# rpl-cmu/bevrender

Measured on AMD Instinct MI355X. Metric: samples/sec fwd+bwd, 6-cam 256x704 BEV-lift+corr, higher is better.
Workload: dtype bf16; 1 GPU; cfg3: 6-cam 256x704 features (64x64x176), 200x200 BEV, C=64 h=2 D=5, L=2 encoder layers (TSA+SCA), T=2 (1 no-grad history frame(s) + 1 fwd+bwd), correlation head with contrastive + lifted-structure losses, AdamW; batch 8 per GPU; backbone/render CNN excluded; global_batch=8, per_gpu_batch=8, parallelism=dp1

## Files before the change

bevrender_amd/csrc/attn_gather_fwd.hip:

```cpp
#include "attn_tap.h"
#include "attn_host.h"

#ifndef BEVR_GATHER_ROWS
#define BEVR_GATHER_ROWS 0
#endif
#ifndef BEVR_GATHER_X3
#define BEVR_GATHER_X3 0
#endif

#include "bevr_prof.h"

BEVR_PROF_DEFINE(gather, 32)

namespace {

constexpr int GT = 32;
constexpr int NT = GT / 32;
constexpr int ROWS = 256;
constexpr int PITCH = 272;
constexpr int WIN_COLS = 28;
constexpr int STRIP_KEYS = WIN_COLS / 2;
template <int NP> struct LdsGn {
  static constexpr int K_IMG = GT * 64, V_IMG = GT * 32, W_IMG = (GT / 16) * 2 * 64 * 16;
  static constexpr int OFF_K = 0;
  static constexpr int OFF_VLO = NP * K_IMG;
  static constexpr int OFF_VHI = OFF_VLO + NP * V_IMG;
  static constexpr int OFF_W = OFF_VHI + NP * V_IMG;
  static constexpr int W_BYTES = NP * W_IMG;
  static constexpr int OFF_OFF = OFF_W + W_BYTES;
  static constexpr int OFF_CT = OFF_OFF + GT * 4;
  static constexpr int OFF_FD = OFF_CT + 16;
  static constexpr int BUF = OFF_FD + WIN_COLS * 8;
  static constexpr int WIN_PLANE = WIN_COLS * PITCH * 4;
  static constexpr int WIN = NP * WIN_PLANE;
  static constexpr int OFF_WIN = 2 * BUF;
  static constexpr int TOTAL = OFF_WIN + 2 * WIN;
};
typedef LdsGn<BEVR_GATHER_X3 ? 2 : 1> LdsG;
static_assert(LdsG::BUF % 16 == 0 && LdsG::WIN % 16 == 0, "16-byte aligned LDS blocks");
static_assert((BEVR_GATHER_X3 ? 1 : 2) * LdsG::TOTAL <= 160 * 1024, "workgroups per CU");
static_assert(LdsG::WIN_PLANE + 2 * QB * 4 < 65536, "the lo plane of a tap is an immediate offset of its hi plane's read");
__device__ __forceinline__ int w_image_pos(int n) {
  const int m = n >> 3, half = (n >> 2) & 1, dd = n & 3;
  return (m * 64 + n + 32 * half) * 16 + dd * 4;
}
__device__ __forceinline__ void barrier_lds() { asm volatile("s_waitcnt lgkmcnt(0)\n\ts_barrier" ::: "memory"); }
__device__ __forceinline__ void wait_vm0() { asm volatile("s_waitcnt vmcnt(0)" ::: "memory"); }
constexpr float RAISE = 40.0f;
constexpr float F16_RAISE = 15.0f;
constexpr float F16_LIFT = 8.0f;
constexpr float F16_PMAX_PER_KEY = 6.103515625e-05f;

template <int V> struct IntC { static constexpr int value = V; };
typedef const char __attribute__((address_space(1)))* gptr_t;
typedef char __attribute__((address_space(3)))* lptr_t;
__device__ __forceinline__ void glds16(const char* src, char* lds_base) {
  __builtin_amdgcn_global_load_lds((gptr_t)src, (lptr_t)lds_base, 16, 0, 0);
}

#if BEVR_DROP
static_assert(BEVR_GATHER_ROWS && !BEVR_GATHER_X3, "the keep mask: the 16-bit row-range kernels");
#define BEVR_GATHER_KERNEL attn_gather_fwd_drop_kernel
#define BEVR_GATHER_ROW_PARAMS , const int row0, const int n_rows, const unsigned drop_thr, const unsigned drop_seed
#define BEVR_GATHER_WAVES_PER_SIMD 4
#elif BEVR_GATHER_X3
#define BEVR_GATHER_KERNEL attn_gather_fwd_x3_kernel
#define BEVR_GATHER_ROW_PARAMS , const int row0, const int n_rows
#define BEVR_GATHER_WAVES_PER_SIMD 2
#elif BEVR_GATHER_ROWS
#define BEVR_GATHER_KERNEL attn_gather_fwd_rows_kernel
#define BEVR_GATHER_ROW_PARAMS , const int row0, const int n_rows
#define BEVR_GATHER_WAVES_PER_SIMD 4
#else
#define BEVR_GATHER_KERNEL attn_gather_fwd_kernel
#define BEVR_GATHER_ROW_PARAMS
#define BEVR_GATHER_WAVES_PER_SIMD 4
#endif
template <int PREC, int NB, bool EXACT, bool DMA>
__global__ __launch_bounds__(512, BEVR_GATHER_WAVES_PER_SIMD) void BEVR_GATHER_KERNEL(
    bevr_attn_desc d, const char* __restrict__ Q, const char* __restrict__ K, const char* __restrict__ V,
    const char* __restrict__ key_ws, const uint32_t* __restrict__ table_pk, const float* __restrict__ mref,
    float* __restrict__ O, float* __restrict__ LSE, int* __restrict__ flags BEVR_GATHER_ROW_PARAMS) {
  constexpr bool BAND = BEVR_GATHER_ROWS != 0;
  constexpr bool X3 = tap_split(PREC);
  static_assert(X3 == (BEVR_GATHER_X3 != 0), "the split mode lives in its own translation unit");
  static_assert(!X3 || BAND, "the split mode takes a row range");
  constexpr int NP = tap_np<PREC>;
  constexpr int ROWB = X3 ? 128 : 64;
  typedef TapHalf<PREC> H16;
#if !BEVR_GATHER_ROWS
  constexpr int row0 = 0, n_rows = 0;
#endif
  typedef LdsG L;
  extern __shared__ __attribute__((aligned(16))) char smem[];

  const int n_ph = d.n_prob * d.heads;
  const int xcd = blockIdx.x & 7, slot = blockIdx.x >> 3;
  const int ph = (slot / d.S) * 8 + xcd;
  if (ph >= n_ph) return;
  const int j = slot % d.S;
  if constexpr (EXACT) {
    if (flags[ph * d.S + j] == 0) return;
  }
  const int prob = ph / d.heads, hd = ph % d.heads;
  const int tid = threadIdx.x, n_wave = blockDim.x >> 6;
  const int wave = __builtin_amdgcn_readfirstlane(tid >> 6), lane = tid & 63;
  const int li = lane & 15, kg = lane >> 4;
  const int Mp = d.S * d.Sp;
  const int nblk = ((BAND ? n_rows : d.S) + QB - 1) / QB;
  const int rows_q = nblk * QB;
  const int row_end = BAND ? row0 + n_rows : d.S;
  const bool to_end = !BAND || row_end == d.S;
  const float rx = (float)(d.Wt - 1) / (2.0f * (float)(d.S - 1));
  const float jrx = (float)j * rx;
  const unsigned smem_base = (unsigned)(size_t)(lptr_t)smem;

  const char* tbl = reinterpret_cast<const char*>(table_pk + (size_t)hd * d.Wp * d.Hp);
  const unsigned lane16 = (unsigned)lane * 16u;
  const size_t tbl_plane = (size_t)d.heads * d.Wp * d.Hp * 4;
  auto fill_one = [&](char* win, int c, int xc, int r0) {
    static_assert(ROWS == 256, "one 16-byte load per lane and column");
    BEVR_ASSERT(c >= 0 && c < WIN_COLS && xc >= 0 && xc < d.Wp && r0 >= 0 && (DMA ? r0 + ROWS <= d.Hp : r0 < d.Hp));
    if constexpr (DMA) {
      const char* sbase = tbl + ((size_t)__builtin_amdgcn_readfirstlane(xc) * d.Hp + __builtin_amdgcn_readfirstlane(r0)) * 4;
      glds16(sbase + lane16, win + (c * PITCH) * 4);
      if constexpr (X3) glds16(sbase + tbl_plane + lane16, win + L::WIN_PLANE + (c * PITCH) * 4);
    } else {
      const int rr = r0 + 4 * lane;
#pragma unroll
      for (int pl = 0; pl < NP; ++pl) {
        const char* src = tbl + pl * tbl_plane + ((size_t)xc * d.Hp + rr) * 4;
        u32x4 v = {0u, 0u, 0u, 0u};
#pragma unroll
        for (int k = 0; k < 4; ++k)
          if (rr + k < d.Hp) v[k] = *reinterpret_cast<const uint32_t*>(src + 4 * k);
        *reinterpret_cast<u32x4*>(win + pl * L::WIN_PLANE + (c * PITCH) * 4 + lane * 16) = v;
      }
    }
  };
  auto fill_share = [&](const int* fd, char* win, int nfill) {
    for (int c = wave; c < nfill; c += n_wave) fill_one(win, c, fd[2 * c], fd[2 * c + 1]);
  };

  for (int i = tid; i < 2 * L::W_BYTES / 16; i += (int)blockDim.x)
    *reinterpret_cast<u32x4*>(smem + (i / (L::W_BYTES / 16)) * L::BUF + L::OFF_W + (i % (L::W_BYTES / 16)) * 16) =
        u32x4{0u, 0u, 0u, 0u};
  if (wave == n_wave - 1) {
    __builtin_amdgcn_s_setprio(3);
    const int pg = prob * d.groups + hd / (d.heads / d.groups);
    const KeyW* kws = reinterpret_cast<const KeyW*>(key_ws) + (size_t)pg * d.Np;
    const StepBox* box = reinterpret_cast<const StepBox*>(key_ws + key_ws_box_offset(d)) + (size_t)pg * (d.Np / 32);
    const char* Kp = K + (size_t)ph * d.Np * ROWB;
    const char* Vp = V + (size_t)ph * d.Np * ROWB;
    const int n_steps = d.Np / GT;

    struct Em {
      unsigned long long sel;
      int step, nfill, fd_xc, fd_r0, koff;
      u32x2 w[NP];
    };
    int step = -1;
    unsigned long long rem = 0ull;
    const int kl = lane & (GT - 1);
    const bool klane = lane < GT;
    KeyW kw_n = kws[kl];
    StepBox sb0_n = box[0], sb1_n = box[NT - 1];
    int ar = 0, xc = 0, x0 = 0, a0w = 0, cols = 0;
    bool fits = false;
    u32x2 w_t[NP];
#pragma unroll
    for (int pl = 0; pl < NP; ++pl) w_t[pl] = u32x2{0u, 0u};
    auto advance = [&](Em& em) -> bool {
      while (rem == 0ull) {
        if (++step >= n_steps) return false;
        const KeyW kw = kw_n;
        const StepBox sb = box_union(sb0_n, sb1_n);
        if (step + 1 < n_steps) {
          kw_n = kws[(size_t)(step + 1) * GT + kl];
          sb0_n = box[NT * (step + 1)];
          sb1_n = box[NT * (step + 1) + NT - 1];
        }
        if (sb.amax < sb.amin) continue;
        const bool live = klane && step * GT + kl < d.N;
        ar = (kw.aoff >> 3) - d.x_off * d.Hp;
        if constexpr (BAND) ar += row0;
        const float tx = jrx + kw.b;
        const float xf = floorf(tx);
        xc = (int)xf + d.x_off;
        const float fx = tx - xf, fy = kw.fy;
        if constexpr (X3) {
          TAP_SPLIT2((1.0f - fx) * (1.0f - fy), (1.0f - fx) * fy, w_t[0][0], w_t[NP - 1][0]);
          TAP_SPLIT2(fx * (1.0f - fy), fx * fy, w_t[0][1], w_t[NP - 1][1]);
        } else {
          w_t[0][0] = H16::pack2((1.0f - fx) * (1.0f - fy), (1.0f - fx) * fy);
          w_t[0][1] = H16::pack2(fx * (1.0f - fy), fx * fy);
        }
        x0 = (int)floorf(jrx + sb.bmin) + d.x_off;
        const int x1 = (int)floorf(jrx + sb.bmax) + 1 + d.x_off;
        cols = x1 - x0 + 1;
        fits = cols <= WIN_COLS && sb.amax - sb.amin + rows_q + 1 <= ROWS;
        a0w = max(0, min(sb.amin + d.y_off + (BAND ? row0 : 0), d.Hp - ROWS));
        rem = __ballot(live);
      }
      em.w[0] = w_t[0];
      if constexpr (X3) em.w[NP - 1] = w_t[NP - 1];
      em.step = step;
      if (fits) {
        em.sel = rem;
        em.koff = ((xc - x0) * PITCH + (ar - a0w)) * 4;
        em.nfill = cols;
        em.fd_xc = x0 + lane;
        em.fd_r0 = a0w;
      } else {
        const int rank = __builtin_popcountll(rem & ((1ull << kl) - 1ull));
        const bool mine = klane && (rem >> kl & 1ull) && rank < STRIP_KEYS;
        em.sel = __ballot(mine);
        const int akw = max(0, min(ar, d.Hp - ROWS));
        em.koff = (2 * rank * PITCH + (ar - akw)) * 4;
        em.nfill = 2 * __builtin_popcountll(em.sel);
        int src = 0;
        {
          unsigned long long t = em.sel;
          for (int k = 0; k < (lane >> 1) && t; ++k) t &= t - 1;
          src = t ? __builtin_ctzll(t) : 0;
        }
        em.fd_xc = __shfl(xc, src) + (lane & 1);
        em.fd_r0 = __shfl(akw, src);
      }
      rem &= ~em.sel;
      return true;
    };
    auto stage = [&](const Em& em, int e, const Em* nxt) {
      char* bb = smem + (e & 1) * L::BUF;
      const size_t n0 = (size_t)em.step * GT;
#pragma unroll
      for (int i = 0; i < GT / 16; ++i) {
        const int n = 16 * i + (lane >> 2), c = (lane & 3) ^ ((n >> 2) & 3);
        if constexpr (X3) {
          const char* src = Kp + (n0 + n) * ROWB + 64 * (c >> 1) + 16 * (c & 1);
          glds16(src, bb + L::OFF_K + i * 1024);
          glds16(src + 32, bb + L::OFF_K + L::K_IMG + i * 1024);
        } else {
          glds16(Kp + (n0 + n) * 64 + 16 * c, bb + L::OFF_K + i * 1024);
        }
      }
#pragma unroll
      for (int i = 0; i < NT; ++i) {
        const int n = 32 * i + (lane >> 1);
        if constexpr (X3) {
          const char* src = Vp + (n0 + n) * ROWB + 16 * (lane & 1);
          glds16(src, bb + L::OFF_VLO + i * 1024);
          glds16(src + 32, bb + L::OFF_VLO + L::V_IMG + i * 1024);
          glds16(src + 64, bb + L::OFF_VHI + i * 1024);
          glds16(src + 96, bb + L::OFF_VHI + L::V_IMG + i * 1024);
        } else {
          glds16(Vp + (n0 + n) * 64 + 16 * (lane & 1), bb + L::OFF_VLO + i * 1024);
          glds16(Vp + (n0 + n) * 64 + 32 + 16 * (lane & 1), bb + L::OFF_VHI + i * 1024);
        }
      }
      if (klane) {
        char* wk = bb + L::OFF_W + (kl >> 4) * 2048 + w_image_pos(kl & 15);
        *reinterpret_cast<uint32_t*>(wk) = em.w[0][0];
        *reinterpret_cast<uint32_t*>(wk + 256) = em.w[0][1];
        if constexpr (X3) {
          *reinterpret_cast<uint32_t*>(wk + L::W_IMG) = em.w[NP - 1][0];
          *reinterpret_cast<uint32_t*>(wk + L::W_IMG + 256) = em.w[NP - 1][1];
        }
        const bool in = em.sel >> kl & 1ull;
        *reinterpret_cast<unsigned*>(bb + L::OFF_OFF + kl * 4) = smem_base + L::OFF_WIN + (e & 1) * L::WIN + (in ? em.koff : 0);
      }
      if (nxt && lane < nxt->nfill) {
        int* fd = reinterpret_cast<int*>(bb + L::OFF_FD);
        fd[2 * lane] = nxt->fd_xc;
        fd[2 * lane + 1] = nxt->fd_r0;
      }
#if BEVR_DROP
      static_assert(NT == 1, "the third dword (live keys 32..63) carries the emission's first key index");
      if (lane == 0)
        *reinterpret_cast<u32x4*>(bb + L::OFF_CT) =
            u32x4{0u, (unsigned)em.sel, (unsigned)(em.step * GT), nxt ? (unsigned)nxt->nfill : 0u};
#else
      if (lane == 0)
        *reinterpret_cast<u32x4*>(bb + L::OFF_CT) =
            u32x4{0u, (unsigned)em.sel, (unsigned)(em.sel >> 32), nxt ? (unsigned)nxt->nfill : 0u};
#endif
    };

    Em cur, nxt;
    advance(cur);
    bool more = advance(nxt);
    {
      int* fd = reinterpret_cast<int*>(smem + L::BUF + L::OFF_FD);
      if (lane < cur.nfill) {
        fd[2 * lane] = cur.fd_xc;
        fd[2 * lane + 1] = cur.fd_r0;
      }
      if (lane == 0) *reinterpret_cast<u32x4*>(smem + L::BUF + L::OFF_CT) = u32x4{0u, 0u, 0u, (unsigned)cur.nfill};
      barrier_lds();
      fill_share(fd, smem + L::OFF_WIN, cur.nfill);
      stage(cur, 0, more ? &nxt : nullptr);
      wait_vm0();
    }
    PROF_ACC(8);
    for (int e = 0;; ++e) {
      PROF_T_FREE(p0);
      barrier_lds();
      PROF_T_FREE(p1);
      if (!more) {
        if (lane == 0) *reinterpret_cast<u32x4*>(smem + ((e + 1) & 1) * L::BUF + L::OFF_CT) = u32x4{4u, 0u, 0u, 0u};
        barrier_lds();
        break;
      }
      cur = nxt;
      {
        char* wn = smem + L::OFF_WIN + ((e + 1) & 1) * L::WIN;
        for (int c = wave; c < cur.nfill; c += n_wave)
          fill_one(wn, c, __builtin_amdgcn_readlane(cur.fd_xc, c), __builtin_amdgcn_readlane(cur.fd_r0, c));
      }
      PROF_T_FREE(p2);
      more = advance(nxt);
      stage(cur, e + 1, more ? &nxt : nullptr);
      PROF_T_FREE(p3);
      wait_vm0();
      PROF_T_FREE(p4);
      PROF_ADD(4, p1 - p0);
      PROF_ADD(6, p2 - p1);
      PROF_ADD(1, p3 - p2);
      PROF_ADD(3, p4 - p3);
      PROF_ADD(5, 1);
    }
    PROF_FLUSH(gather, 0, lane == 0);
    return;
  }

  const int blk0 = wave * NB;
  const int qb = prob / d.q_div;
  TapOp<NP> qf[NB];
  f32x4 o_lo[NB], o_hi[NB];
  f32x4 negm[NB];
  f32x4 lacc[NB];
  float pmx[NB];
#if BEVR_DROP
  uint32_t hrow[NB];
#endif
  const unsigned qoff0 = (unsigned)(blk0 * QB + li) * 4u + (unsigned)(kg & 1) * (PITCH * 4u);
#pragma unroll
  for (int nb = 0; nb < NB; ++nb) {
    const int row = (BAND ? row0 : 0) + min(blk0 + nb, nblk - 1) * QB + li;
    const size_t mcol = (size_t)j * d.Sp + row;
    if constexpr (X3)
      qf[nb] = tap_ld<NP>(Q + (((size_t)qb * d.heads + hd) * Mp + mcol) * ROWB + 64 * (kg >> 1) + 16 * (kg & 1), 32);
    else
      qf[nb].p[0] = __builtin_bit_cast(
          bf16x8, *reinterpret_cast<const u32x4*>(Q + ((((size_t)qb * d.heads + hd) * Mp + mcol) * 32 + 8 * kg) * 2));
    o_lo[nb] = o_hi[nb] = f32x4{0.f, 0.f, 0.f, 0.f};
    const float mr = EXACT ? 0.f : mref[(size_t)ph * Mp + mcol];
    negm[nb] = f32x4{-mr, -mr, -mr, -mr};
    lacc[nb] = f32x4{0.f, 0.f, 0.f, 0.f};
    pmx[nb] = 0.f;
#if BEVR_DROP
    hrow[nb] = bevr_drop_row(drop_seed, (uint32_t)ph, (uint32_t)mcol);
#endif
  }
  const uint32_t one2 = H16::pack2(1.0f, 1.0f);
  const bf16x8 ones = __builtin_bit_cast(bf16x8, u32x4{one2, one2, one2, one2});
  const int t_off = (4 * kg + (li >> 2)) * 32 + (lane & 3) * 8;
  const int k_off = li * 64 + 16 * (kg ^ (li >> 2));
  typedef const uint32_t __attribute__((address_space(3)))* lds_u32p;
  typedef const volatile uint32_t __attribute__((address_space(3)))* vlds_u32p;

  {
    barrier_lds();
    const int nf0 = __builtin_amdgcn_readfirstlane((int)reinterpret_cast<const u32x4*>(smem + L::BUF + L::OFF_CT)[0][3]);
    fill_share(reinterpret_cast<const int*>(smem + L::BUF + L::OFF_FD), smem + L::OFF_WIN, nf0);
    wait_vm0();
  }
  bool first = true;
  PROF_ACC(8);
  PROF_T_FREE(cprev);
  auto sweep = [&](auto off1_c) {
  constexpr int OFF1 = decltype(off1_c)::value;
  constexpr int NBX = (NB == 2 && OFF1 == 0) ? 1 : NB;
  for (int e = 0;; ++e) {
    PROF_T_FREE(c0);
    barrier_lds();
    PROF_T_FREE(c1);
    PROF_ADD(0, c1 - c0);
    PROF_ADD(4, c0 - cprev);
    PROF_ADD(5, 1);
    PROF_SET(cprev, c1);
    const char* bb = smem + (e & 1) * L::BUF;
    const u32x4 ct = *reinterpret_cast<const u32x4*>(bb + L::OFF_CT);
    if (__builtin_amdgcn_readfirstlane((int)ct[0]) & 4) break;
    fill_share(reinterpret_cast<const int*>(bb + L::OFF_FD), smem + L::OFF_WIN + ((e + 1) & 1) * L::WIN,
               __builtin_amdgcn_readfirstlane((int)ct[3]));
#pragma unroll 1
    for (int t = 0; t < NT; ++t) {
      const unsigned livem = (unsigned)__builtin_amdgcn_readfirstlane((int)(t ? ct[2] : ct[1]));
      const TapOp<NP> vlo = tap_ld_tr<NP>(bb + L::OFF_VLO + t * 1024 + t_off, 512, L::V_IMG);
      const TapOp<NP> vhi = tap_ld_tr<NP>(bb + L::OFF_VHI + t * 1024 + t_off, 512, L::V_IMG);
      u32x4 pw[NB][NP];
#if BEVR_DROP
      u32x4 km[NB];
      const uint32_t kh0 = ((uint32_t)__builtin_amdgcn_readfirstlane((int)ct[2]) + 4u * (uint32_t)kg) * 0xC2B2AE3Du;
#endif
#pragma unroll
      for (int s2 = 0; s2 < 2; ++s2) {
        const int kb = 32 * t + 16 * s2;
        const TapOp<NP> kf = tap_ld<NP>(bb + L::OFF_K + kb * 64 + k_off, L::K_IMG);
        const TapOp<NP> wa0 = tap_ld<NP>(bb + L::OFF_W + kb * 128 + lane * 16, L::W_IMG);
        const TapOp<NP> wa1 = tap_ld<NP>(bb + L::OFF_W + kb * 128 + 1024 + lane * 16, L::W_IMG);
        const int kq = 4 * (kg >> 1);
        const u32x4 oc0 = *reinterpret_cast<const u32x4*>(bb + L::OFF_OFF + (kb + kq) * 4);
        const u32x4 oc1 = *reinterpret_cast<const u32x4*>(bb + L::OFF_OFF + (kb + 8 + kq) * 4);
        f32x4 sv[NB];
        u32x4 g0[NB][NP], g1[NB][NP];
#pragma unroll
        for (int dd = 0; dd < 4; ++dd) {
          const lds_u32p p0 = (lds_u32p)(uintptr_t)(oc0[dd] + qoff0), p1 = (lds_u32p)(uintptr_t)(oc1[dd] + qoff0);
#ifdef BEVR_DEBUG
          {
            const unsigned w0 = smem_base + L::OFF_WIN + (e & 1) * L::WIN, last = (unsigned)((NBX - 1) * OFF1) * 4u;
            BEVR_ASSERT(oc0[dd] + qoff0 >= w0 && oc0[dd] + qoff0 + last + 4u <= w0 + L::WIN_PLANE);
            BEVR_ASSERT(oc1[dd] + qoff0 >= w0 && oc1[dd] + qoff0 + last + 4u <= w0 + L::WIN_PLANE);
          }
#endif
          if constexpr (X3) {
#pragma unroll
            for (int nb = 0; nb < NBX; ++nb) {
              g0[nb][0][dd] = ((vlds_u32p)p0)[nb * OFF1];
              g1[nb][0][dd] = ((vlds_u32p)p1)[nb * OFF1];
              g0[nb][NP - 1][dd] = ((vlds_u32p)p0)[nb * OFF1 + L::WIN_PLANE / 4];
              g1[nb][NP - 1][dd] = ((vlds_u32p)p1)[nb * OFF1 + L::WIN_PLANE / 4];
            }
          } else
#pragma unroll
          for (int nb = 0; nb < NBX; ++nb) {
            if (nb == 0) {
              g0[nb][0][dd] = p0[0];
              g1[nb][0][dd] = p1[0];
            } else {
              g0[nb][0][dd] = ((vlds_u32p)p0)[nb * OFF1];
              g1[nb][0][dd] = ((vlds_u32p)p1)[nb * OFF1];
            }
          }
        }
#pragma unroll
        for (int nb = 0; nb < NBX; ++nb) {
          sv[nb] = tap_mm<PREC>(kf, qf[nb], negm[nb]);
          sv[nb] = tap_mm<PREC>(wa0, tap_op(g0[nb]), sv[nb]);
          sv[nb] = tap_mm<PREC>(wa1, tap_op(g1[nb]), sv[nb]);
        }
        if ((livem >> (16 * s2) & 0xffffu) != 0xffffu) {
#pragma unroll
          for (int nb = 0; nb < NBX; ++nb)
#pragma unroll
            for (int r = 0; r < 4; ++r)
              if (!(livem >> (16 * s2 + 4 * kg + r) & 1u)) sv[nb][r] = -1.0e30f;
        }
#pragma unroll
        for (int nb = 0; nb < NBX; ++nb) {
          if constexpr (EXACT) {
            const float tm = fmaxf(fmaxf(sv[nb][0], sv[nb][1]), fmaxf(sv[nb][2], sv[nb][3]));
            constexpr float RAISE_P = PREC == BEVR_PREC_F16 ? F16_RAISE : RAISE;
            if (first || __any(tm > RAISE_P)) {
              float tx = fmaxf(tm, __shfl_xor(tm, 16));
              tx = fmaxf(tx, __shfl_xor(tx, 32));
              if constexpr (PREC == BEVR_PREC_F16) tx -= F16_LIFT;
              const float delta = first ? tx : fmaxf(tx, 0.f);
              const float al = first ? 1.0f : fast_exp2(-delta);
              negm[nb] -= delta;
              o_lo[nb] *= al;
              o_hi[nb] *= al;
              lacc[nb] *= al;
              pmx[nb] *= al;
              sv[nb] -= delta;
              if (s2 == 1) {
#pragma unroll
                for (int k = 0; k < 2; ++k) {
                  if constexpr (X3)
                    tap_pack2<PREC>((H16::lo(pw[nb][0][k]) + H16::lo(pw[nb][NP - 1][k])) * al,
                                    (H16::hi(pw[nb][0][k]) + H16::hi(pw[nb][NP - 1][k])) * al, k, pw[nb]);
                  else
                    pw[nb][0][k] = H16::pack2(H16::lo(pw[nb][0][k]) * al, H16::hi(pw[nb][0][k]) * al);
                }
              }
            }
          }
          const f32x2 pa = {fast_exp2(sv[nb][0]), fast_exp2(sv[nb][1])}, pb2 = {fast_exp2(sv[nb][2]), fast_exp2(sv[nb][3])};
          if constexpr (X3) {
            tap_pack2<PREC>(pa[0], pa[1], 2 * s2, pw[nb]);
            tap_pack2<PREC>(pb2[0], pb2[1], 2 * s2 + 1, pw[nb]);
          } else {
            pw[nb][0][2 * s2] = H16::pack2(pa[0], pa[1]);
            pw[nb][0][2 * s2 + 1] = H16::pack2(pb2[0], pb2[1]);
          }
          pmx[nb] = fmaxf(fmaxf(fmaxf(pmx[nb], pa[0]), pa[1]), fmaxf(pb2[0], pb2[1]));
#if BEVR_DROP
#pragma unroll
          for (int k = 0; k < 2; ++k) {
            const uint32_t kn = kh0 + (uint32_t)(16 * s2 + 2 * k) * 0xC2B2AE3Du;
            const bool k0 = (bevr_drop_mix(hrow[nb] ^ kn) >> 16) >= drop_thr;
            const bool k1 = (bevr_drop_mix(hrow[nb] ^ (kn + 0xC2B2AE3Du)) >> 16) >= drop_thr;
            km[nb][2 * s2 + k] = (k0 ? 0xffffu : 0u) | (k1 ? 0xffff0000u : 0u);
          }
#endif
        }
        if constexpr (EXACT) first = false;
      }
#pragma unroll
      for (int nb = 0; nb < NBX; ++nb) {
        const TapOp<NP> pb = tap_op(pw[nb]);
#if BEVR_DROP
        const u32x4 pk[NP] = {pw[nb][0] & km[nb]};
        const TapOp<NP> pkb = tap_op(pk);
        o_lo[nb] = tap_mm<PREC>(vlo, pkb, o_lo[nb]);
        o_hi[nb] = tap_mm<PREC>(vhi, pkb, o_hi[nb]);
#else
        o_lo[nb] = tap_mm<PREC>(vlo, pb, o_lo[nb]);
        o_hi[nb] = tap_mm<PREC>(vhi, pb, o_hi[nb]);
#endif
#pragma unroll
        for (int pl = NP - 1; pl >= 0; --pl) lacc[nb] = mfma16<PREC>(ones, pb.p[pl], lacc[nb]);
      }
    }
    PROF_T_FREE(c2);
    PROF_ADD(1, c2 - c1);
    wait_vm0();
    PROF_T_FREE(c3);
    PROF_ADD(2, c3 - c2);
  }
  };
  if constexpr (NB == 2) {
    if (blk0 + 1 < nblk) sweep(IntC<QB>{});
    else sweep(IntC<0>{});
  } else {
    sweep(IntC<0>{});
  }
  PROF_FLUSH(gather, wave ? 16 : 8, lane == 0 && (wave == 0 || wave == 3));

  bool bad = false;
#pragma unroll
  for (int nb = 0; nb < NB; ++nb) {
    if (blk0 + nb >= nblk) continue;
    const float l = lacc[nb][0];
    float pm = fmaxf(pmx[nb], __shfl_xor(pmx[nb], 16));
    pm = fmaxf(pm, __shfl_xor(pm, 32));
    const int row = (BAND ? row0 : 0) + (blk0 + nb) * QB + li;
    if (!EXACT && row < row_end && !(l >= 7.9e-31f && l < 3.0e38f)) bad = true;
    if constexpr (!EXACT && PREC == BEVR_PREC_F16) {
      if (row < row_end && !(pm >= (float)d.N * F16_PMAX_PER_KEY)) bad = true;
    }
    if (BAND && !to_end && row >= row_end) continue;
#if BEVR_DROP
    const float inv = (65536.0f / (65536.0f - (float)drop_thr)) / l;
#else
    const float inv = 1.0f / l;
#endif
    const size_t mq = (size_t)ph * Mp + (size_t)j * d.Sp + row;
    float* orow = O + mq * 32;
    *reinterpret_cast<f32x4*>(orow + 4 * kg) = o_lo[nb] * inv;
    *reinterpret_cast<f32x4*>(orow + 16 + 4 * kg) = o_hi[nb] * inv;
    if (kg == 0) {
      const float lg = __log2f(l);
      const int n_copy = (to_end && blk0 + nb == nblk - 1) ? (d.Sp - row + QB - 1) / QB : 1;
      for (int k = 0; k < n_copy; ++k) {
        float lse0 = lg - negm[nb][0];
        if constexpr (BAND || PREC == BEVR_PREC_F16) {
          constexpr float PAD_FLOOR = PREC == BEVR_PREC_F16 ? 70.0f : -36.0f;
          if (k > 0) lse0 = fmaxf(lse0, mref[mq + k * QB] + PAD_FLOOR);
        }
        LSE[mq + k * QB] = lse0;
        LSE[(size_t)n_ph * Mp + mq + k * QB] = __log2f(pm) - lg;
      }
    }
  }
  if constexpr (!EXACT) {
    if (__any(bad) && lane == 0) flags[ph * d.S + j] = 1;
  }
}

template <int PREC>
int launch(const bevr_attn_desc& d, const void* Q, const void* K, const void* V, const void* key_ws,
           const void* table_pk, const float* mref, float* O, float* LSE, int* flags, int row0, int n_rows,
           hipStream_t st BEVR_DROP_PARAMS) {
  typedef LdsG L;
  const int n_ph = d.n_prob * d.heads;
  const int grid = ((n_ph + 7) / 8) * 8 * d.S;
  const int nblk = ((BEVR_GATHER_ROWS ? n_rows : d.S) + QB - 1) / QB;
  if (nblk * QB + 1 > ROWS || nblk > 14) return BEVR_E_SHAPE;
  const int nb = nblk <= 7 ? 1 : 2;
  const int n_cw = (nblk + nb - 1) / nb;
  const dim3 block(64 * (n_cw + 1));
#if BEVR_DROP
#define BEVR_GATHER_ROW_ARGS , row0, n_rows, drop_thr, drop_seed
#elif BEVR_GATHER_ROWS
#define BEVR_GATHER_ROW_ARGS , row0, n_rows
#else
#define BEVR_GATHER_ROW_ARGS
#endif
#define BEVR_GATHER_LAUNCH_(NB_, EX_, DMA_)                                                                          \
  hipLaunchKernelGGL((BEVR_GATHER_KERNEL<PREC, NB_, EX_, DMA_>), dim3(grid), block, L::TOTAL, st, d,                \
                     (const char*)Q, (const char*)K, (const char*)V, (const char*)key_ws, (const uint32_t*)table_pk, \
                     mref, O, LSE, flags BEVR_GATHER_ROW_ARGS)
#if BEVR_GATHER_X3
#define BEVR_GATHER_LAUNCH(NB_, EX_, DMA_)                                                                           \
  do {                                                                                                               \
    const int ea = bevr_raise_dynamic_lds<&BEVR_GATHER_KERNEL<PREC, NB_, EX_, DMA_>>(L::TOTAL);                      \
    if (ea) return ea;                                                                                               \
    BEVR_GATHER_LAUNCH_(NB_, EX_, DMA_);                                                                             \
  } while (0)
#else
#define BEVR_GATHER_LAUNCH(NB_, EX_, DMA_) BEVR_GATHER_LAUNCH_(NB_, EX_, DMA_)
#endif
  const bool dma = d.Hp >= ROWS;
  for (int ex = 0; ex < 2; ++ex) {
    if (nb == 1) {
      if (dma) { if (ex) BEVR_GATHER_LAUNCH(1, true, true); else BEVR_GATHER_LAUNCH(1, false, true); }
      else { if (ex) BEVR_GATHER_LAUNCH(1, true, false); else BEVR_GATHER_LAUNCH(1, false, false); }
    } else {
      if (dma) { if (ex) BEVR_GATHER_LAUNCH(2, true, true); else BEVR_GATHER_LAUNCH(2, false, true); }
      else { if (ex) BEVR_GATHER_LAUNCH(2, true, false); else BEVR_GATHER_LAUNCH(2, false, false); }
    }
    const int rc = (int)hipGetLastError();
    if (rc) return rc;
  }
#undef BEVR_GATHER_LAUNCH
#undef BEVR_GATHER_LAUNCH_
  return BEVR_OK;
}

template <int... PRECS>
int run(const bevr_attn_desc* d, const void* Q, const void* K, const void* V, const void* key_ws, const void* table_pk,
        const float* mref, float* O, float* LSE, int* flags, int row0, int n_rows, void* stream BEVR_DROP_PARAMS) {
  int rc = bevr_check_desc(d);
  if (rc) return rc;
  if (!Q || !K || !V || !key_ws || !table_pk || !mref || !O || !LSE || !flags) return BEVR_E_NULL;
  if (!bevr_aligned16(Q) || !bevr_aligned16(K) || !bevr_aligned16(V) || !bevr_aligned16(O) || !bevr_aligned16(key_ws))
    return BEVR_E_ALIGN;
  return bevr_for_precision<PRECS...>(d->precision, [&](auto P) {
    if (BEVR_GATHER_ROWS && (row0 < 0 || row0 % QB != 0 || n_rows < 1 || n_rows > 14 * QB || n_rows > d->S - row0))
      return (int)BEVR_E_SHAPE;
    return launch<P()>(*d, Q, K, V, key_ws, table_pk, mref, O, LSE, flags, row0, n_rows, (hipStream_t)stream BEVR_DROP_ARGS);
  });
}

}

#if BEVR_DROP
extern "C" int bevr_attn_gather_fwd_dropout(const bevr_attn_desc* d, const void* Q, const void* K, const void* V,
                                            const void* key_ws, const void* table_pk, const float* mref, float* O,
                                            float* LSE, int* flags, int row0, int n_rows, unsigned drop_thr,
                                            unsigned drop_seed, void* stream) {
  if (drop_thr >= 65536u) return BEVR_E_SHAPE;
  return run<BEVR_PREC_BF16, BEVR_PREC_F16>(d, Q, K, V, key_ws, table_pk, mref, O, LSE, flags, row0, n_rows, stream,
                                            drop_thr, drop_seed);
}
#elif BEVR_GATHER_X3
extern "C" int bevr_attn_gather_fwd_x3(const bevr_attn_desc* d, const void* Q, const void* K, const void* V,
                                       const void* key_ws, const void* table_pk2, const float* mref, float* O,
                                       float* LSE, int* flags, int row0, int n_rows, void* stream) {
  return run<BEVR_PREC_BF16X3>(d, Q, K, V, key_ws, table_pk2, mref, O, LSE, flags, row0, n_rows, stream);
}
#elif BEVR_GATHER_ROWS
extern "C" int bevr_attn_gather_fwd_rows(const bevr_attn_desc* d, const void* Q, const void* K, const void* V,
                                         const void* key_ws, const void* table_pk, const float* mref, float* O,
                                         float* LSE, int* flags, int row0, int n_rows, void* stream) {
  return run<BEVR_PREC_BF16, BEVR_PREC_F16>(d, Q, K, V, key_ws, table_pk, mref, O, LSE, flags, row0, n_rows, stream);
}
#else
extern "C" int bevr_attn_gather_fwd(const bevr_attn_desc* d, const void* Q, const void* K, const void* V,
                                    const void* key_ws, const void* table_pk, const float* mref, float* O, float* LSE,
                                    int* flags, void* stream) {
  return run<BEVR_PREC_BF16, BEVR_PREC_F16>(d, Q, K, V, key_ws, table_pk, mref, O, LSE, flags, 0, 0, stream);
}
#endif
```

bevrender_amd/csrc/attn_host.h:

```cpp
#pragma once
#include <mutex>
#include <type_traits>
#include "bevr_common.h"

template <int P0, int... PRECS, typename F>
int bevr_for_precision(int precision, F&& f) {
  if (precision == P0) return f(std::integral_constant<int, P0>());
  if constexpr (sizeof...(PRECS) > 0) return bevr_for_precision<PRECS...>(precision, f);
  return BEVR_E_PRECISION;
}

constexpr int BEVR_MAX_DEVICES = 64;
class BevrPerDevice {
  std::mutex lock_[BEVR_MAX_DEVICES];
  int value_[BEVR_MAX_DEVICES] = {};
 public:
  template <typename F> int get(F&& query) {
    int dev = 0;
    if (hipGetDevice(&dev) != hipSuccess || dev < 0 || dev >= BEVR_MAX_DEVICES) return 0;
    std::lock_guard<std::mutex> hold(lock_[dev]);
    if (value_[dev] == 0) value_[dev] = query(dev);
    return value_[dev];
  }
};

static inline int bevr_cu_count() {
  static BevrPerDevice cus;
  return cus.get([](int dev) {
    int n = 0;
    return hipDeviceGetAttribute(&n, hipDeviceAttributeMultiprocessorCount, dev) == hipSuccess && n > 0 ? n : 0;
  });
}

template <auto KERN>
int bevr_resident_workgroups(int threads, size_t lds) {
  static BevrPerDevice resident;
  return resident.get([&](int) {
    int per_cu = 0;
    if (hipOccupancyMaxActiveBlocksPerMultiprocessor(&per_cu, KERN, threads, lds) != hipSuccess) return 0;
    return bevr_cu_count() * per_cu;
  });
}

template <auto KERN>
int bevr_raise_dynamic_lds(int bytes) {
  static BevrPerDevice raised;
  hipError_t e = hipErrorInvalidDevice;
  const int done = raised.get([&](int) {
    e = hipFuncSetAttribute(reinterpret_cast<const void*>(KERN), hipFuncAttributeMaxDynamicSharedMemorySize, bytes);
    return e == hipSuccess ? 1 : 0;
  });
  return done ? 0 : (int)e;
}

constexpr int LIST_HEAD = 4;
static inline size_t bevr_list_bytes(size_t n_units) { return (LIST_HEAD + n_units) * sizeof(int); }
static inline int bevr_list_clear(int* list, hipStream_t st) { return (int)hipMemsetAsync(list, 0, LIST_HEAD * sizeof(int), st); }
template <auto KERN>
int bevr_list_workgroups(int max_workgroups, int threads, size_t lds) {
  const int resident = bevr_resident_workgroups<KERN>(threads, lds);
  return max_workgroups > 0 && max_workgroups < resident ? max_workgroups : resident;
}
```

Measured before the change: 5.908 samples/s.

## Stagger gather-forward waves by deferring the PV matmul into the next emission

In the non-row-range gather forward kernel, waves 4-7 now run a 'late' sweep variant. It saves the V operands and probabilities (or, in the non-exact path, the raw scores) of each tile and does the exp, PV MFMA and row-sum accumulation at the start of the next emission, after the barrier. This offsets the MFMA-heavy phase of half the waves against the score and exp phase of the other half, so matrix and vector units overlap better within the workgroup. The cost is extra registers to hold the pending tile, which may hurt occupancy. The mode is on by default and can be disabled with BEVR_STAGGER=0.

```diff
diff --git a/bevrender_amd/csrc/attn_gather_fwd.hip b/bevrender_amd/csrc/attn_gather_fwd.hip
--- a/bevrender_amd/csrc/attn_gather_fwd.hip
+++ b/bevrender_amd/csrc/attn_gather_fwd.hip
@@ -73,9 +73,10 @@
 #define BEVR_GATHER_WAVES_PER_SIMD 4
 #else
 #define BEVR_GATHER_KERNEL attn_gather_fwd_kernel
-#define BEVR_GATHER_ROW_PARAMS
+#define BEVR_GATHER_ROW_PARAMS , const int stagger
 #define BEVR_GATHER_WAVES_PER_SIMD 4
 #endif
+#define BEVR_GATHER_STAGGER (!BEVR_GATHER_ROWS)
 template <int PREC, int NB, bool EXACT, bool DMA>
 __global__ __launch_bounds__(512, BEVR_GATHER_WAVES_PER_SIMD) void BEVR_GATHER_KERNEL(
     bevr_attn_desc d, const char* __restrict__ Q, const char* __restrict__ K, const char* __restrict__ V,
@@ -378,9 +379,38 @@
   bool first = true;
   PROF_ACC(8);
   PROF_T_FREE(cprev);
-  auto sweep = [&](auto off1_c) {
+  auto sweep = [&](auto off1_c, auto late_c) {
   constexpr int OFF1 = decltype(off1_c)::value;
+  constexpr bool LATE = decltype(late_c)::value != 0;
   constexpr int NBX = (NB == 2 && OFF1 == 0) ? 1 : NB;
+  constexpr bool LATE_EXP = LATE && !EXACT;
+  f32x4 pend_sv[2][NB];
+  auto pv_tail = [&](const TapOp<NP>& tvlo, const TapOp<NP>& tvhi, u32x4 (&tpw)[NB][NP]) {
+    if constexpr (LATE_EXP) {
+#pragma unroll
+      for (int s2 = 0; s2 < 2; ++s2)
+#pragma unroll
+      for (int nb = 0; nb < NBX; ++nb) {
+        const f32x4 p = {fast_exp2(pend_sv[s2][nb][0]), fast_exp2(pend_sv[s2][nb][1]), fast_exp2(pend_sv[s2][nb][2]),
+                         fast_exp2(pend_sv[s2][nb][3])};
+        tpw[nb][0][2 * s2] = H16::pack2(p[0], p[1]);
+        tpw[nb][0][2 * s2 + 1] = H16::pack2(p[2], p[3]);
+        pmx[nb] = fmaxf(fmaxf(fmaxf(pmx[nb], p[0]), p[1]), fmaxf(p[2], p[3]));
+      }
+    }
+#pragma unroll
+    for (int nb = 0; nb < NBX; ++nb) {
+      const TapOp<NP> pb = tap_op(tpw[nb]);
+      o_lo[nb] = tap_mm<PREC>(tvlo, pb, o_lo[nb]);
+      o_hi[nb] = tap_mm<PREC>(tvhi, pb, o_hi[nb]);
+#pragma unroll
+      for (int pl = NP - 1; pl >= 0; --pl) lacc[nb] = mfma16<PREC>(ones, pb.p[pl], lacc[nb]);
+    }
+  };
+  static_assert(!LATE || (NT == 1 && !BEVR_DROP), "the pending tail is the emission's one tile, without a keep mask");
+  u32x4 pend_pw[NB][NP];
+  TapOp<NP> pend_vlo, pend_vhi;
+  bool pend = false;
   for (int e = 0;; ++e) {
     PROF_T_FREE(c0);
     barrier_lds();
@@ -394,6 +424,9 @@
     if (__builtin_amdgcn_readfirstlane((int)ct[0]) & 4) break;
     fill_share(reinterpret_cast<const int*>(bb + L::OFF_FD), smem + L::OFF_WIN + ((e + 1) & 1) * L::WIN,
                __builtin_amdgcn_readfirstlane((int)ct[3]));
+    if constexpr (LATE) {
+      if (pend) pv_tail(pend_vlo, pend_vhi, pend_pw);
+    }
 #pragma unroll 1
     for (int t = 0; t < NT; ++t) {
       const unsigned livem = (unsigned)__builtin_amdgcn_readfirstlane((int)(t ? ct[2] : ct[1]));
@@ -487,6 +520,10 @@
               }
             }
           }
+          if constexpr (LATE_EXP) {
+            pend_sv[s2][nb] = sv[nb];
+            continue;
+          }
           const f32x2 pa = {fast_exp2(sv[nb][0]), fast_exp2(sv[nb][1])}, pb2 = {fast_exp2(sv[nb][2]), fast_exp2(sv[nb][3])};
           if constexpr (X3) {
             tap_pack2<PREC>(pa[0], pa[1], 2 * s2, pw[nb]);
@@ -508,21 +545,34 @@
         }
         if constexpr (EXACT) first = false;
       }
+#if BEVR_DROP
 #pragma unroll
       for (int nb = 0; nb < NBX; ++nb) {
         const TapOp<NP> pb = tap_op(pw[nb]);
-#if BEVR_DROP
         const u32x4 pk[NP] = {pw[nb][0] & km[nb]};
         const TapOp<NP> pkb = tap_op(pk);
         o_lo[nb] = tap_mm<PREC>(vlo, pkb, o_lo[nb]);
         o_hi[nb] = tap_mm<PREC>(vhi, pkb, o_hi[nb]);
+#pragma unroll
+        for (int pl = NP - 1; pl >= 0; --pl) lacc[nb] = mfma16<PREC>(ones, pb.p[pl], lacc[nb]);
+      }
 #else
-        o_lo[nb] = tap_mm<PREC>(vlo, pb, o_lo[nb]);
-        o_hi[nb] = tap_mm<PREC>(vhi, pb, o_hi[nb]);
-#endif
-#pragma unroll
-        for (int pl = NP - 1; pl >= 0; --pl) lacc[nb] = mfma16<PREC>(ones, pb.p[pl], lacc[nb]);
-      }
+      if constexpr (LATE_EXP) {
+        pend_vlo = vlo;
+        pend_vhi = vhi;
+        pend = true;
+      } else if constexpr (LATE) {
+#pragma unroll
+        for (int nb = 0; nb < NBX; ++nb)
+#pragma unroll
+          for (int pl = 0; pl < NP; ++pl) pend_pw[nb][pl] = pw[nb][pl];
+        pend_vlo = vlo;
+        pend_vhi = vhi;
+        pend = true;
+      } else {
+        pv_tail(vlo, vhi, pw);
+      }
+#endif
     }
     PROF_T_FREE(c2);
     PROF_ADD(1, c2 - c1);
@@ -530,12 +580,25 @@
     PROF_T_FREE(c3);
     PROF_ADD(2, c3 - c2);
   }
+  if constexpr (LATE) {
+    if (pend) pv_tail(pend_vlo, pend_vhi, pend_pw);
+  }
   };
+#if BEVR_GATHER_STAGGER
+  if (stagger && wave >= 4) {
+    if constexpr (NB == 2) {
+      if (blk0 + 1 < nblk) sweep(IntC<QB>{}, IntC<1>{});
+      else sweep(IntC<0>{}, IntC<1>{});
+    } else {
+      sweep(IntC<0>{}, IntC<1>{});
+    }
+  } else
+#endif
   if constexpr (NB == 2) {
-    if (blk0 + 1 < nblk) sweep(IntC<QB>{});
-    else sweep(IntC<0>{});
+    if (blk0 + 1 < nblk) sweep(IntC<QB>{}, IntC<0>{});
+    else sweep(IntC<0>{}, IntC<0>{});
   } else {
-    sweep(IntC<0>{});
+    sweep(IntC<0>{}, IntC<0>{});
   }
   PROF_FLUSH(gather, wave ? 16 : 8, lane == 0 && (wave == 0 || wave == 3));
 
@@ -597,7 +660,8 @@
 #elif BEVR_GATHER_ROWS
 #define BEVR_GATHER_ROW_ARGS , row0, n_rows
 #else
-#define BEVR_GATHER_ROW_ARGS
+#define BEVR_GATHER_ROW_ARGS , stagger
+  const int stagger = bevr_stagger();
 #endif
 #define BEVR_GATHER_LAUNCH_(NB_, EX_, DMA_)                                                                          \
   hipLaunchKernelGGL((BEVR_GATHER_KERNEL<PREC, NB_, EX_, DMA_>), dim3(grid), block, L::TOTAL, st, d,                \
diff --git a/bevrender_amd/csrc/attn_host.h b/bevrender_amd/csrc/attn_host.h
--- a/bevrender_amd/csrc/attn_host.h
+++ b/bevrender_amd/csrc/attn_host.h
@@ -1,4 +1,5 @@
 #pragma once
+#include <cstdlib>
 #include <mutex>
 #include <type_traits>
 #include "bevr_common.h"
@@ -53,6 +54,11 @@
   return done ? 0 : (int)e;
 }
 
+static inline int bevr_stagger() {
+  const char* s = getenv("BEVR_STAGGER");
+  return !(s && s[0] == '0' && s[1] == 0);
+}
+
 constexpr int LIST_HEAD = 4;
 static inline size_t bevr_list_bytes(size_t n_units) { return (LIST_HEAD + n_units) * sizeof(int); }
 static inline int bevr_list_clear(int* list, hipStream_t st) { return (int)hipMemsetAsync(list, 0, LIST_HEAD * sizeof(int), st); }
```

New measurement: 5.954 samples/s (median of 6 runs). No clear change (+0.8%).
